# Jeremy-Cleland/hmer-img2latex

Measured on AMD Instinct MI355X. Metric: decoded LaTeX tokens/sec at batch 256, 320x64 imgs, seq 150, higher is better.
Workload: dtype f32

## Files before the change

hmer-img2latex_amd/csrc/conv_bf16x3.hip:

```cpp
#include <stdlib.h>

#include "common.h"

namespace {

#include "bf16_split.inc.h"

typedef float f32x16 __attribute__((ext_vector_type(16)));

constexpr int CH = 16;
constexpr int CO_BLK = 64;
constexpr int W_SLAB_U4 = 9 * 3 * 2 * CO_BLK;
constexpr int W_PHASE_U4 = W_SLAB_U4 / 3;

template <int WX> struct Tile3 {
    static constexpr int TR = (4 / WX) * 4, TC = WX * 16;
    static constexpr int IR = TR + 2, IC = TC + 2;
    static constexpr int ICP = WX == 2 ? 36 : (WX == 1 ? 20 : 68);
    static constexpr int ROW16 = 2 * ICP;
    static constexpr int IN_U4 = 3 * IR * ROW16;
};

constexpr unsigned FIX_HDR = 64;
constexpr unsigned FIX_CAP = 1u << 20;
constexpr float FIX_TOL = 0x1p-13f;

__device__ __forceinline__ void pool_window(float a0, float a1, float a2, float a3, float bv, float& outv, int& bi, bool& near) {
    float best = a0;
    bi = 0;
    if (a1 > best) { best = a1; bi = 1; }
    if (a2 > best) { best = a2; bi = 2; }
    if (a3 > best) { best = a3; bi = 3; }
    const float pre = best + bv;
    outv = fmaxf(pre, 0.f);
    const float scale = fmaxf(fmaxf(fabsf(best), fabsf(bv)), 1e-30f);
    const float thr = FIX_TOL * scale;
    const float d0 = best - a0, d1 = best - a1, d2 = best - a2, d3 = best - a3;
    const bool tie = (d0 > 0.f && d0 <= thr) || (d1 > 0.f && d1 <= thr) || (d2 > 0.f && d2 <= thr) || (d3 > 0.f && d3 <= thr);
    near = fabsf(pre) <= thr || (tie && pre > 0.f);
}
__device__ __forceinline__ void fix_append(unsigned* fix, size_t o) {
    const unsigned at = atomicAdd(fix, 1u);
    if (at < FIX_CAP) fix[FIX_HDR + at] = (unsigned)o;
}

__global__ void conv_pack3_kernel(const float* __restrict__ w, bf16_t* __restrict__ wp, int Cin, int Cout, int n_chunks,
                                  size_t total, int flip, unsigned* __restrict__ fix) {
    const size_t idx = (size_t)blockIdx.x * blockDim.x + threadIdx.x;
    if (idx == 0 && fix) fix[0] = 0;
    if (idx >= total) return;
    size_t r = idx;
    const int j = (int)(r % 8); r /= 8;
    const int co_l = (int)(r % CO_BLK); r /= CO_BLK;
    const int lh = (int)(r % 2); r /= 2;
    const int tap = (int)(r % 9); r /= 9;
    const int chunk = (int)(r % n_chunks);
    const int cb = (int)(r / n_chunks);
    const int co = cb * CO_BLK + co_l, ci = chunk * CH + 8 * lh + j;
    const float v = (co < Cout && ci < Cin) ? (flip ? w[((size_t)ci * Cout + co) * 9 + (8 - tap)] : w[((size_t)co * Cin + ci) * 9 + tap]) : 0.f;
    bf16_t s[3];
    split3(v, s[0], s[1], s[2]);
    const size_t slab = ((size_t)cb * n_chunks + chunk) * (size_t)W_SLAB_U4 * 8;
#pragma unroll
    for (int sp = 0; sp < 3; ++sp)
        wp[slab + ((((size_t)tap * 3 + sp) * 2 + lh) * CO_BLK + co_l) * 8 + j] = s[sp];
}

template <int WX, bool FULL = false, bool AM = false, int NT = 2>
__global__ __launch_bounds__(256, 2) void conv3x3_bf16x3_kernel(
    const float* __restrict__ x, const bf16_t* __restrict__ wpack, const float* __restrict__ bias,
    float* __restrict__ y, unsigned char* __restrict__ amax, int Cin, int H, int W, int Cout, int Hp, int Wp,
    int tiles_x, int n_chunks, int tiles_per_img, int n_items, int items_per_wg, unsigned* __restrict__ fix) {
    typedef Tile3<WX> TL;
    constexpr int PR = TL::TR / 2, PC = TL::TC / 2;
    constexpr bool LO = FULL && NT == 1;
    __shared__ __attribute__((aligned(16))) uint4 in_s[TL::IN_U4];
    __shared__ __attribute__((aligned(16))) uint4 w_s[W_PHASE_U4];
    __shared__ float out_s[CO_BLK * 65];
    __shared__ unsigned char am_s[AM ? CO_BLK * 68 : 4];

    const int tid = threadIdx.x, lane = tid & 63, wave = tid >> 6;
    const int wy = wave / WX, wx = wave % WX;
    constexpr int CO_W = 32 * NT;
    const int co_blocks_g = (Cout + CO_W - 1) / CO_W;
    const int lin = blockIdx.x, within = lin % (8 * co_blocks_g);
    const int cb = within >> 3;
    const int walk = (lin / (8 * co_blocks_g)) * 8 + (within & 7);
    const int i = lane & 31, h = lane >> 5;
    const int dx = i & 1, dy = (i >> 1) & 1, pp = i >> 2;
    const int a_base = ((wy * 4 + dy) * 2 + h) * TL::ICP + wx * 16 + 2 * pp + dx;
    const int b_base = h * CO_BLK + i + (NT == 1 ? (cb & 1) * 32 : 0);
    const uint4* wp_cb = reinterpret_cast<const uint4*>(wpack) + (size_t)(NT == 1 ? cb >> 1 : cb) * n_chunks * W_SLAB_U4;
    const int HW = H * W;

    constexpr int NP = TL::IR * 2 * TL::IC;
    constexpr int NE = (NP + 255) / 256;
    constexpr int NWV = (W_PHASE_U4 + 255) / 256;
    constexpr int SPLIT_U4 = TL::IR * TL::ROW16;
    int loff[NE], p_r[NE], p_col[NE], p_lh[NE];
#pragma unroll
    for (int e = 0; e < NE; ++e) {
        const int idx = tid + e * 256;
        p_col[e] = idx % TL::IC;
        p_lh[e] = (idx / TL::IC) & 1;
        p_r[e] = idx / (2 * TL::IC);
        loff[e] = idx < NP ? (p_r[e] * 2 + p_lh[e]) * TL::ICP + p_col[e] : -1;
    }
    const float* f_xb = x;
    int goff[NE];
    unsigned okmask = 0;
    auto setup_fetch = [&](int item) {
        const int fb = item / tiles_per_img, ft = item - fb * tiles_per_img;
        const int fty = ft / tiles_x, ftx = ft - fty * tiles_x;
        const int fy0 = fty * TL::TR, fx0 = ftx * TL::TC;
        f_xb = x + (size_t)fb * Cin * HW;
        okmask = 0;
#pragma unroll
        for (int e = 0; e < NE; ++e) {
            const int iy = fy0 - 1 + p_r[e], ix = fx0 - 1 + p_col[e];
            goff[e] = (8 * p_lh[e] * H + iy) * W + ix;
            if (loff[e] >= 0 && iy >= 0 && iy < H && ix >= 0 && ix < W) okmask |= 1u << e;
        }
    };
    float xin[NE][8];
    uint4 win[NWV];
    auto fetch_x = [&](int chunk) {
        const float* xc = f_xb + (size_t)chunk * CH * HW;
#pragma unroll
        for (int e = 0; e < NE; ++e) {
            const bool ok = (okmask >> e) & 1u;
#pragma unroll
            for (int j = 0; j < 8; ++j) xin[e][j] = ok ? xc[goff[e] + j * HW] : 0.f;
        }
    };
    auto fetch_w = [&](int phase) {
        const uint4* wsrc = wp_cb + (size_t)phase * W_PHASE_U4;
#pragma unroll
        for (int e = 0; e < NWV; ++e) {
            const int idx = tid + e * 256;
            win[e] = idx < W_PHASE_U4 ? wsrc[idx] : make_uint4(0, 0, 0, 0);
        }
    };
    auto commit_x = [&]() {
#pragma unroll
        for (int e = 0; e < NE; ++e) {
            if (loff[e] >= 0) {
                unsigned s[3][4];
#pragma unroll
                for (int j = 0; j < 4; ++j) split3_pair(xin[e][2 * j], xin[e][2 * j + 1], s[0][j], s[1][j], s[2][j]);
#pragma unroll
                for (int sp = 0; sp < 3; ++sp)
                    in_s[loff[e] + sp * SPLIT_U4] = make_uint4(s[sp][0], s[sp][1], s[sp][2], s[sp][3]);
            }
        }
    };
    auto commit_w = [&]() {
#pragma unroll
        for (int e = 0; e < NWV; ++e) {
            const int idx = tid + e * 256;
            if (idx < W_PHASE_U4) w_s[idx] = win[e];
        }
    };

    const int n_phases = 3 * n_chunks;
    const int it0 = walk * items_per_wg, it_end = min(it0 + items_per_wg, n_items);
    if (it0 >= n_items) return;
    setup_fetch(it0);
    fetch_x(0);
    fetch_w(0);
    for (int it = it0; it < it_end; ++it) {
        const int b = it / tiles_per_img, tl = it - b * tiles_per_img;
        const int ty = tl / tiles_x, tx = tl - ty * tiles_x;
        const int y0 = ty * TL::TR, x0 = tx * TL::TC;
        f32x16 acc[2][NT];
        f32x16 acc_lo[LO ? 2 : 1];
#pragma unroll
        for (int m = 0; m < 2; ++m)
#pragma unroll
            for (int n = 0; n < NT; ++n)
#pragma unroll
                for (int r = 0; r < 16; ++r) acc[m][n][r] = 0.f;
        if constexpr (LO) {
#pragma unroll
            for (int m = 0; m < 2; ++m)
#pragma unroll
                for (int r = 0; r < 16; ++r) acc_lo[m][r] = 0.f;
        }

        for (int chunk = 0; chunk < n_chunks; ++chunk) {
#pragma unroll
            for (int ky = 0; ky < 3; ++ky) {
                __syncthreads();
                if (ky == 0) commit_x();
                commit_w();
                __syncthreads();
                if (chunk * 3 + ky + 1 < n_phases) fetch_w(chunk * 3 + ky + 1);
                else if (it + 1 < it_end) fetch_w(0);
                if (ky == 0) {
                    if (chunk + 1 < n_chunks) fetch_x(chunk + 1);
                    else if (it + 1 < it_end) { setup_fetch(it + 1); fetch_x(0); }
                }
#pragma unroll
                for (int kx = 0; kx < 3; ++kx) {
                    i16x8_t a[2][3], bw[NT][3];
#pragma unroll
                    for (int m = 0; m < 2; ++m)
#pragma unroll
                        for (int sp = 0; sp < 3; ++sp) {
                            const uint4 t = in_s[a_base + (sp * TL::IR + m * 2 + ky) * TL::ROW16 + kx];
                            a[m][sp] = *reinterpret_cast<const i16x8_t*>(&t);
                        }
#pragma unroll
                    for (int n = 0; n < NT; ++n)
#pragma unroll
                        for (int sp = 0; sp < 3; ++sp) {
                            const uint4 t = w_s[b_base + ((kx * 3 + sp) * 2) * CO_BLK + n * 32];
                            bw[n][sp] = *reinterpret_cast<const i16x8_t*>(&t);
                        }
                    constexpr int TI[6] = {0, 1, 2, 0, 1, 0}, TJ[6] = {2, 1, 0, 1, 0, 0};
#pragma unroll
                    for (int t = 0; t < 6; ++t)
#pragma unroll
                        for (int m = 0; m < 2; ++m)
#pragma unroll
                            for (int n = 0; n < NT; ++n) {
                                if constexpr (LO) {
                                    f32x16& dst = t < 5 ? acc_lo[m] : acc[m][n];
                                    dst = __builtin_amdgcn_mfma_f32_32x32x16_bf16(a[m][TI[t]], bw[n][TJ[t]], dst, 0, 0, 0);
                                } else {
                                    acc[m][n] = __builtin_amdgcn_mfma_f32_32x32x16_bf16(a[m][TI[t]], bw[n][TJ[t]], acc[m][n], 0, 0, 0);
                                }
                            }
                }
            }
        }

        const int py0 = y0 >> 1, px0 = x0 >> 1;
        if constexpr (LO) {
#pragma unroll
            for (int m = 0; m < 2; ++m) acc[m][0] += acc_lo[m];
        }
        if constexpr (FULL) {
#pragma unroll
            for (int n = 0; n < NT; ++n) {
                const int co = cb * CO_W + n * 32 + i;
                if (co >= Cout) continue;
#pragma unroll
                for (int m = 0; m < 2; ++m) {
                    const int py = py0 + wy * 2 + m;
#pragma unroll
                    for (int q = 0; q < 4; ++q) {
                        const int px = px0 + wx * 8 + 2 * q + h;
#pragma unroll
                        for (int ry = 0; ry < 2; ++ry) {
                            const int Y = 2 * py + ry, X = 2 * px;
                            if (Y < H && X + 1 < W)
                                *reinterpret_cast<float2*>(y + (((size_t)b * Cout + co) * H + Y) * W + X) =
                                    make_float2(acc[m][n][4 * q + 2 * ry], acc[m][n][4 * q + 2 * ry + 1]);
                        }
                    }
                }
            }
            continue;
        }
        if ((Wp & 3) == 0 && py0 + PR <= Hp && px0 + PC <= Wp && (cb + 1) * CO_BLK <= Cout) {
#pragma unroll
            for (int n = 0; n < NT; ++n) {
                const float bv = bias[cb * CO_BLK + n * 32 + i];
#pragma unroll
                for (int m = 0; m < 2; ++m)
#pragma unroll
                    for (int q = 0; q < 4; ++q) {
                        const int pos = (wy * 2 + m) * PC + wx * 8 + 2 * q + h;
                        if constexpr (AM) {
                            float ov;
                            int bi;
                            bool near;
                            pool_window(acc[m][n][4 * q], acc[m][n][4 * q + 1], acc[m][n][4 * q + 2], acc[m][n][4 * q + 3], bv, ov, bi, near);
                            out_s[(n * 32 + i) * 65 + pos] = ov;
                            am_s[(n * 32 + i) * 68 + pos] = (unsigned char)bi;
                            if (near && fix)
                                fix_append(fix, (((size_t)b * Cout + cb * CO_BLK + n * 32 + i) * Hp + py0 + wy * 2 + m) * Wp + px0 + wx * 8 + 2 * q + h);
                        } else {
                            const float v = fmaxf(fmaxf(acc[m][n][4 * q], acc[m][n][4 * q + 1]),
                                                  fmaxf(acc[m][n][4 * q + 2], acc[m][n][4 * q + 3])) + bv;
                            out_s[(n * 32 + i) * 65 + pos] = fmaxf(v, 0.f);
                        }
                    }
            }
            __syncthreads();
            for (int idx = tid; idx < CO_BLK * 16; idx += 256) {
                constexpr int XG = PC / 4;
                const int x4 = idx % XG, py = (idx / XG) % PR, co_l = idx >> 4;
                const float* sp = &out_s[co_l * 65 + py * PC + 4 * x4];
                const size_t o = (((size_t)b * Cout + cb * CO_BLK + co_l) * Hp + py0 + py) * Wp + px0 + 4 * x4;
                *reinterpret_cast<float4*>(y + o) = make_float4(sp[0], sp[1], sp[2], sp[3]);
                if constexpr (AM) *reinterpret_cast<uchar4*>(amax + o) = *reinterpret_cast<const uchar4*>(&am_s[co_l * 68 + py * PC + 4 * x4]);
            }
            continue;
        }
#pragma unroll
        for (int n = 0; n < NT; ++n) {
            const int co = cb * CO_BLK + n * 32 + i;
            if (co >= Cout) continue;
            const float bv = bias[co];
#pragma unroll
            for (int m = 0; m < 2; ++m) {
                const int py = py0 + wy * 2 + m;
                if (py >= Hp) continue;
                const size_t rowoff = (((size_t)b * Cout + co) * Hp + py) * Wp;
#pragma unroll
                for (int q = 0; q < 4; ++q) {
                    const int px = px0 + wx * 8 + 2 * q + h;
                    float ov;
                    int bi;
                    bool near;
                    pool_window(acc[m][n][4 * q], acc[m][n][4 * q + 1], acc[m][n][4 * q + 2], acc[m][n][4 * q + 3], bv, ov, bi, near);
                    if (px < Wp) {
                        y[rowoff + px] = ov;
                        if (amax) amax[rowoff + px] = (unsigned char)bi;
                        if (AM && near && fix) fix_append(fix, rowoff + px);
                    }
                }
            }
        }
    }
}


template <int CIN, bool AM = false>
__global__ __launch_bounds__(256, 4) void conv3x3_smallk_bf16x3_kernel(
    const float* __restrict__ x, const float* __restrict__ w, const float* __restrict__ bias, float* __restrict__ y,
    unsigned char* __restrict__ amax, int H, int W, int Cout, int Hp, int Wp, int tiles_x, int tiles_per_part,
    unsigned* __restrict__ fix) {
    constexpr int RS = 48;
    constexpr int PLANE = 10 * RS;
    __shared__ __attribute__((aligned(16))) uint2 img[3 * PLANE];
    __shared__ float out_s[32 * 65];
    __shared__ unsigned char am_s[AM ? 32 * 68 : 4];

    const int tid = threadIdx.x, lane = tid & 63, wave = tid >> 6;
    const int wy = wave >> 1, wx = wave & 1;
    const int i = lane & 31, h = lane >> 5;
    const int cbs = (Cout + 31) / 32;
    const int cb = blockIdx.x % cbs, b = blockIdx.z;
    const int tx_begin = (blockIdx.x / cbs) * tiles_per_part, tx_end = min(tiles_x, tx_begin + tiles_per_part);
    const int y0 = blockIdx.y * 8;

    i16x8_t bw[3][3];
    {
        const int co = cb * 32 + i;
#pragma unroll
        for (int s = 0; s < 3; ++s) {
            unsigned pk[3][4];
#pragma unroll
            for (int j = 0; j < 4; ++j) {
                const int tap = 4 * s + 2 * h + (j >> 1), c0 = 2 * (j & 1);
                const bool okt = tap < 9 && co < Cout;
                const float v0 = (okt && c0 < CIN) ? w[((size_t)co * CIN + c0) * 9 + tap] : 0.f;
                const float v1 = (okt && c0 + 1 < CIN) ? w[((size_t)co * CIN + c0 + 1) * 9 + tap] : 0.f;
                split3_pair(v0, v1, pk[0][j], pk[1][j], pk[2][j]);
            }
#pragma unroll
            for (int sp = 0; sp < 3; ++sp) {
                const uint4 t = make_uint4(pk[sp][0], pk[sp][1], pk[sp][2], pk[sp][3]);
                bw[s][sp] = *reinterpret_cast<const i16x8_t*>(&t);
            }
        }
    }
    const float bv = (cb * 32 + i < Cout) ? bias[cb * 32 + i] : 0.f;

    const int pbase = (wy * 4 + ((i >> 1) & 1)) * RS + wx * 16 + 2 * (i >> 2) + (i & 1);
    int aoff[3][2];
#pragma unroll
    for (int s = 0; s < 3; ++s)
#pragma unroll
        for (int e = 0; e < 2; ++e) {
            const int tap = min(4 * s + 2 * h + e, 8);
            aoff[s][e] = pbase + (tap / 3) * RS + (tap % 3);
        }

    const float* xb = x + (size_t)b * CIN * H * W;
    const size_t HW = (size_t)H * W;
    int q_lds[2], q_col[2];
    long q_goff[2];
    bool q_rowok[2];
#pragma unroll
    for (int e = 0; e < 2; ++e) {
        const int q = tid + e * 256;
        const int r = q / 34, col = q - r * 34;
        const int iy = y0 - 1 + r;
        q_lds[e] = q < 340 ? r * RS + col : -1;
        q_col[e] = col - 1;
        q_rowok[e] = q < 340 && iy >= 0 && iy < H;
        q_goff[e] = (long)iy * W + col - 1;
    }
    float pin[2][CIN];
    auto fetch = [&](int tx) {
        const int x0 = tx * 32;
#pragma unroll
        for (int e = 0; e < 2; ++e) {
            const int ix = x0 + q_col[e];
            const bool ok = q_rowok[e] && ix >= 0 && ix < W;
#pragma unroll
            for (int c = 0; c < CIN; ++c) pin[e][c] = ok ? xb[c * HW + q_goff[e] + x0] : 0.f;
        }
    };
    fetch(tx_begin);
    for (int tx = tx_begin; tx < tx_end; ++tx) {
#pragma unroll
        for (int e = 0; e < 2; ++e) {
            if (q_lds[e] >= 0) {
                unsigned p0[3], p1[3];
                split3_pair(pin[e][0], CIN > 1 ? pin[e][CIN > 1 ? 1 : 0] : 0.f, p0[0], p0[1], p0[2]);
                split3_pair(CIN > 2 ? pin[e][CIN > 2 ? 2 : 0] : 0.f, 0.f, p1[0], p1[1], p1[2]);
#pragma unroll
                for (int sp = 0; sp < 3; ++sp) img[sp * PLANE + q_lds[e]] = make_uint2(p0[sp], p1[sp]);
            }
        }
        __syncthreads();
        if (tx + 1 < tx_end) fetch(tx + 1);
#pragma unroll 1
        for (int m = 0; m < 2; ++m) {
            f32x16 acc;
#pragma unroll
            for (int r = 0; r < 16; ++r) acc[r] = 0.f;
            constexpr int TI[5] = {0, 1, 2, 0, 1}, TJ[5] = {2, 1, 0, 1, 0};
            i16x8_t a0[3];
#pragma unroll
            for (int s = 0; s < 3; ++s) {
                i16x8_t a[3];
#pragma unroll
                for (int sp = 0; sp < 3; ++sp) {
                    const uint2 t0 = img[sp * PLANE + m * 2 * RS + aoff[s][0]];
                    const uint2 t1 = img[sp * PLANE + m * 2 * RS + aoff[s][1]];
                    const uint4 t = make_uint4(t0.x, t0.y, t1.x, t1.y);
                    a[sp] = *reinterpret_cast<const i16x8_t*>(&t);
                }
                a0[s] = a[0];
#pragma unroll
                for (int t = 0; t < 5; ++t)
                    acc = __builtin_amdgcn_mfma_f32_32x32x16_bf16(a[TI[t]], bw[s][TJ[t]], acc, 0, 0, 0);
            }
#pragma unroll
            for (int s = 0; s < 3; ++s) acc = __builtin_amdgcn_mfma_f32_32x32x16_bf16(a0[s], bw[s][0], acc, 0, 0, 0);
#pragma unroll
            for (int q = 0; q < 4; ++q) {
                const int pos = (wy * 2 + m) * 16 + wx * 8 + 2 * q + h;
                if constexpr (AM) {
                    float ov;
                    int bi;
                    bool near;
                    pool_window(acc[4 * q], acc[4 * q + 1], acc[4 * q + 2], acc[4 * q + 3], bv, ov, bi, near);
                    out_s[i * 65 + pos] = ov;
                    am_s[i * 68 + pos] = (unsigned char)bi;
                    const int fpy = (y0 >> 1) + wy * 2 + m, fpx = tx * 16 + wx * 8 + 2 * q + h;
                    if (near && fix && cb * 32 + i < Cout && fpy < Hp && fpx < Wp)
                        fix_append(fix, (((size_t)b * Cout + cb * 32 + i) * Hp + fpy) * Wp + fpx);
                } else {
                    const float v = fmaxf(fmaxf(acc[4 * q], acc[4 * q + 1]), fmaxf(acc[4 * q + 2], acc[4 * q + 3])) + bv;
                    out_s[i * 65 + pos] = fmaxf(v, 0.f);
                }
            }
        }
        __syncthreads();
        const int py0 = y0 >> 1, px0 = tx * 16;
        if ((Wp & 3) == 0 && py0 + 4 <= Hp && px0 + 16 <= Wp && (cb + 1) * 32 <= Cout) {
            for (int idx = tid; idx < 32 * 16; idx += 256) {
                const int x4 = idx & 3, py = (idx >> 2) & 3, c = idx >> 4;
                const float* sp = &out_s[c * 65 + py * 16 + 4 * x4];
                const size_t o = (((size_t)b * Cout + cb * 32 + c) * Hp + py0 + py) * Wp + px0 + 4 * x4;
                *reinterpret_cast<float4*>(y + o) = make_float4(sp[0], sp[1], sp[2], sp[3]);
                if constexpr (AM) *reinterpret_cast<uchar4*>(amax + o) = *reinterpret_cast<const uchar4*>(&am_s[c * 68 + py * 16 + 4 * x4]);
            }
        } else {
            for (int idx = tid; idx < 32 * 64; idx += 256) {
                const int px = idx & 15, py = (idx >> 4) & 3, c = idx >> 6;
                if (cb * 32 + c < Cout && py0 + py < Hp && px0 + px < Wp) {
                    const size_t o = (((size_t)b * Cout + cb * 32 + c) * Hp + py0 + py) * Wp + px0 + px;
                    y[o] = out_s[c * 65 + py * 16 + px];
                    if constexpr (AM) amax[o] = am_s[c * 68 + py * 16 + px];
                }
            }
        }
    }
}

__global__ __launch_bounds__(256) void conv_pool_fixup_kernel(const float* __restrict__ x, const float* __restrict__ w,
                                                              const float* __restrict__ bias, float* __restrict__ y,
                                                              unsigned char* __restrict__ amax, const unsigned* __restrict__ fix,
                                                              int Cin, int H, int W, int Cout, int Hp, int Wp) {
    const unsigned n = min(fix[0], FIX_CAP);
    const int lane = threadIdx.x & 63;
    for (unsigned e = blockIdx.x * 4 + (threadIdx.x >> 6); e < n; e += gridDim.x * 4) {
        const unsigned o = fix[FIX_HDR + e];
        const int px = (int)(o % Wp), py = (int)((o / Wp) % Hp);
        const int co = (int)((o / ((unsigned)Wp * Hp)) % Cout), b = (int)(o / ((unsigned)Wp * Hp * Cout));
        float s[4] = {0.f, 0.f, 0.f, 0.f};
        for (int ci = lane; ci < Cin; ci += 64) {
            const float* xp = x + ((size_t)b * Cin + ci) * H * W;
            const float* wp = w + ((size_t)co * Cin + ci) * 9;
            float win[4][4];
#pragma unroll
            for (int r = 0; r < 4; ++r)
#pragma unroll
                for (int c = 0; c < 4; ++c) {
                    const int iy = 2 * py - 1 + r, ix = 2 * px - 1 + c;
                    win[r][c] = (iy >= 0 && iy < H && ix >= 0 && ix < W) ? xp[(size_t)iy * W + ix] : 0.f;
                }
#pragma unroll
            for (int ky = 0; ky < 3; ++ky)
#pragma unroll
                for (int kx = 0; kx < 3; ++kx) {
                    const float wv = wp[ky * 3 + kx];
#pragma unroll
                    for (int q = 0; q < 4; ++q) s[q] = fmaf(win[(q >> 1) + ky][(q & 1) + kx], wv, s[q]);
                }
        }
#pragma unroll
        for (int q = 0; q < 4; ++q)
#pragma unroll
            for (int off = 32; off >= 1; off >>= 1) s[q] += __shfl_xor(s[q], off);
        if (lane == 0) {
            float best = s[0];
            int bi = 0;
#pragma unroll
            for (int q = 1; q < 4; ++q)
                if (s[q] > best) { best = s[q]; bi = q; }
            y[o] = fmaxf(best + bias[co], 0.f);
            amax[o] = (unsigned char)bi;
        }
    }
}

}

bool i2l_conv_bf16x3_applicable(int Cin, int Cout) {
    return Cin % CH == 0 && Cout % CO_BLK == 0;
}
bool i2l_conv_bf16x3_full_applicable(int Cin, int Cout) {
    return Cin % CH == 0 && (Cout % CO_BLK == 0 || Cout == 32);
}

size_t i2l_conv_bf16x3_workspace_bytes(int Cin, int Cout) {
    return i2l_align((size_t)((Cout + CO_BLK - 1) / CO_BLK) * (Cin / CH) * W_SLAB_U4 * 16);
}
size_t i2l_conv_fixlist_bytes(void) { return i2l_align((size_t)(FIX_HDR + FIX_CAP) * sizeof(unsigned)); }

namespace {
int launch_fixup(const float* x, const float* w, const float* bias, float* y, unsigned char* amax, const unsigned* fix,
                 int B, int Cin, int H, int W, int Cout, hipStream_t s) {
    if ((size_t)B * Cout * (H / 2) * (W / 2) > 0xffffffffull) return I2L_ERR_UNSUPPORTED;
    hipLaunchKernelGGL(conv_pool_fixup_kernel, dim3(512), dim3(256), 0, s, x, w, bias, y, amax, fix, Cin, H, W, Cout, H / 2, W / 2);
    I2L_CHECK_LAUNCH();
    return I2L_OK;
}
}

int i2l_conv_bf16x3_run(const float* x, const float* w, const float* bias, float* y, unsigned char* amax, int B, int Cin,
                        int H, int W, int Cout, void* workspace, size_t workspace_bytes, hipStream_t s, int full,
                        int weights_packed) {
    if (full && ((H | W) & 1)) return I2L_ERR_UNSUPPORTED;
    const size_t pack_bytes = i2l_conv_bf16x3_workspace_bytes(Cin, Cout);
    if (workspace_bytes < pack_bytes + (amax ? i2l_conv_fixlist_bytes() : 0) || !workspace) return I2L_ERR_WORKSPACE;
    unsigned* fix = amax ? reinterpret_cast<unsigned*>(static_cast<char*>(workspace) + pack_bytes) : nullptr;
    if (amax && (size_t)B * Cout * (H / 2) * (W / 2) > 0xffffffffull) return I2L_ERR_UNSUPPORTED;
    const int Hp = H / 2, Wp = W / 2;
    const int n_chunks = Cin / CH, co_blocks = (Cout + CO_BLK - 1) / CO_BLK;
    if (Cout % CO_BLK != 0 && !(full && Cout == 32)) return I2L_ERR_UNSUPPORTED;
    bf16_t* wp = static_cast<bf16_t*>(workspace);
    const size_t total = (size_t)co_blocks * n_chunks * 9 * 2 * CO_BLK * 8;
    if (!(weights_packed && !amax && !full))
    hipLaunchKernelGGL(conv_pack3_kernel, dim3((unsigned)((total + 255) / 256)), dim3(256), 0, s, w, wp, Cin, Cout,
                       n_chunks, total, full ? 1 : 0, fix);
    I2L_CHECK_LAUNCH();
    const int rows = 2 * Hp, cols = 2 * Wp;
    int wx = 2;
    long bestw = -1;
    const int cand[3] = {2, 1, 4};
    for (int c = 0; c < 3; ++c) {
        const int tr = (4 / cand[c]) * 4, tc = cand[c] * 16;
        const long cover = (long)i2l_cdiv(rows, tr) * tr * i2l_cdiv(cols, tc) * tc;
        if (bestw < 0 || cover < bestw) { bestw = cover; wx = cand[c]; }
    }
    const int tr = (4 / wx) * 4, tc = wx * 16;
    const int tiles_x = i2l_cdiv(cols, tc), tiles_y = i2l_cdiv(rows, tr);
    const int tiles_per_img = tiles_x * tiles_y;
    const long long n_items_ll = (long long)tiles_per_img * B;
    if (n_items_ll > 0x7fffffffll) return I2L_ERR_UNSUPPORTED;
    const int n_items = (int)n_items_ll;
    const int wg_blocks = full ? (Cout + 31) / 32 : co_blocks;
    int items_per_wg = (int)((n_items_ll * wg_blocks + 511) / 512);
    if (n_items_ll * wg_blocks <= 768) items_per_wg = 1;
    if (items_per_wg < 1) items_per_wg = 1;
    const int walks = i2l_cdiv(n_items, items_per_wg);
    dim3 grid((unsigned)(i2l_cdiv(walks, 8) * 8 * wg_blocks));
#define I2L_LAUNCH3(WXV)                                                                                              \
    do {                                                                                                              \
        if (full)                                                                                                     \
            hipLaunchKernelGGL((conv3x3_bf16x3_kernel<WXV, true, false, 1>), grid, dim3(256), 0, s, x, (const bf16_t*)wp, bias, y, \
                               amax, Cin, H, W, Cout, Hp, Wp, tiles_x, n_chunks, tiles_per_img, n_items, items_per_wg, fix); \
        else if (amax)                                                                                                \
            hipLaunchKernelGGL((conv3x3_bf16x3_kernel<WXV, false, true>), grid, dim3(256), 0, s, x, (const bf16_t*)wp, bias, y, \
                               amax, Cin, H, W, Cout, Hp, Wp, tiles_x, n_chunks, tiles_per_img, n_items, items_per_wg, fix); \
        else                                                                                                          \
            hipLaunchKernelGGL((conv3x3_bf16x3_kernel<WXV, false>), grid, dim3(256), 0, s, x, (const bf16_t*)wp, bias, y, \
                               amax, Cin, H, W, Cout, Hp, Wp, tiles_x, n_chunks, tiles_per_img, n_items, items_per_wg, fix); \
    } while (0)
    if (wx == 2) I2L_LAUNCH3(2);
    else if (wx == 1) I2L_LAUNCH3(1);
    else I2L_LAUNCH3(4);
#undef I2L_LAUNCH3
    I2L_CHECK_LAUNCH();
    if (amax) return launch_fixup(x, w, bias, y, amax, fix, B, Cin, H, W, Cout, s);
    return I2L_OK;
}

bool i2l_conv_smallk_applicable(int Cin, int Cout) {
    return Cin >= 1 && Cin <= 3 && Cout % 32 == 0;
}

int i2l_conv_smallk_run(const float* x, const float* w, const float* bias, float* y, unsigned char* amax, int B, int Cin,
                        int H, int W, int Cout, void* workspace, size_t workspace_bytes, hipStream_t s) {
    const int Hp = H / 2, Wp = W / 2;
    unsigned* fix = nullptr;
    if (amax) {
        if (!workspace || workspace_bytes < i2l_conv_fixlist_bytes()) return I2L_ERR_WORKSPACE;
        if ((size_t)B * Cout * Hp * Wp > 0xffffffffull) return I2L_ERR_UNSUPPORTED;
        fix = static_cast<unsigned*>(workspace);
        if (hipMemsetAsync(fix, 0, sizeof(unsigned), s) != hipSuccess) return I2L_ERR_LAUNCH;
    }
    const int tiles_x = i2l_cdiv(2 * Wp, 32), bands = i2l_cdiv(2 * Hp, 8);
    if (bands > 65535 || B > 65535) return I2L_ERR_UNSUPPORTED;
    int parts = 1;
    while (parts < tiles_x && (long)(Cout / 32) * bands * B * parts < 1536) ++parts;
    const int tiles_per_part = i2l_cdiv(tiles_x, parts);
    parts = i2l_cdiv(tiles_x, tiles_per_part);
    dim3 grid((Cout / 32) * parts, bands, B);
#define I2L_LAUNCH_SK(C, A) hipLaunchKernelGGL((conv3x3_smallk_bf16x3_kernel<C, A>), grid, dim3(256), 0, s, x, w, bias, y, amax, H, W, Cout, Hp, Wp, tiles_x, tiles_per_part, fix)
    if (amax) {
        if (Cin == 1) I2L_LAUNCH_SK(1, true);
        else if (Cin == 2) I2L_LAUNCH_SK(2, true);
        else I2L_LAUNCH_SK(3, true);
    } else {
        if (Cin == 1) I2L_LAUNCH_SK(1, false);
        else if (Cin == 2) I2L_LAUNCH_SK(2, false);
        else I2L_LAUNCH_SK(3, false);
    }
#undef I2L_LAUNCH_SK
    I2L_CHECK_LAUNCH();
    if (amax) return launch_fixup(x, w, bias, y, amax, fix, B, Cin, H, W, Cout, s);
    return I2L_OK;
}
```

Baseline: 41.22 million.

## Double-buffer first-layer small-K conv tiles and overlap staging with MFMA compute

Splits the small-K bf16x3 conv into separate argmax and plain kernels. The plain kernel double-buffers the LDS input image and the output staging tile. It commits the next tile and stores the previous tile's pooled outputs between the two MFMA m-tiles, with sched barriers, so it needs one __syncthreads per tile instead of two. Input addressing switches to 32-bit byte offsets to cut address math, and a guard is added for tensors that would overflow it. The cost is roughly double the LDS per block, which may lower occupancy below the launch-bounds target of 4 blocks.

```diff
diff --git a/hmer-img2latex_amd/csrc/conv_bf16x3.hip b/hmer-img2latex_amd/csrc/conv_bf16x3.hip
--- a/hmer-img2latex_amd/csrc/conv_bf16x3.hip
+++ b/hmer-img2latex_amd/csrc/conv_bf16x3.hip
@@ -328,16 +328,125 @@
 }
 
 
-template <int CIN, bool AM = false>
-__global__ __launch_bounds__(256, 4) void conv3x3_smallk_bf16x3_kernel(
+constexpr int SK_RS = 48;
+constexpr int SK_PLANE = 10 * SK_RS;
+constexpr int SK_IMG = 3 * SK_PLANE;
+constexpr int SK_OUT = 32 * 65;
+
+template <int CIN>
+__device__ __forceinline__ void smallk_filter_bank(const float* __restrict__ w, int co, int Cout, int h, i16x8_t (&bw)[3][3]) {
+#pragma unroll
+    for (int s = 0; s < 3; ++s) {
+        unsigned pk[3][4];
+#pragma unroll
+        for (int j = 0; j < 4; ++j) {
+            const int tap = 4 * s + 2 * h + (j >> 1), c0 = 2 * (j & 1);
+            const bool okt = tap < 9 && co < Cout;
+            const float v0 = (okt && c0 < CIN) ? w[((size_t)co * CIN + c0) * 9 + tap] : 0.f;
+            const float v1 = (okt && c0 + 1 < CIN) ? w[((size_t)co * CIN + c0 + 1) * 9 + tap] : 0.f;
+            split3_pair(v0, v1, pk[0][j], pk[1][j], pk[2][j]);
+        }
+#pragma unroll
+        for (int sp = 0; sp < 3; ++sp) {
+            const uint4 t = make_uint4(pk[sp][0], pk[sp][1], pk[sp][2], pk[sp][3]);
+            bw[s][sp] = *reinterpret_cast<const i16x8_t*>(&t);
+        }
+    }
+}
+
+__device__ __forceinline__ void smallk_a_offsets(int wy, int wx, int i, int h, int (&aoff)[3][2]) {
+    const int pbase = (wy * 4 + ((i >> 1) & 1)) * SK_RS + wx * 16 + 2 * (i >> 2) + (i & 1);
+#pragma unroll
+    for (int s = 0; s < 3; ++s)
+#pragma unroll
+        for (int e = 0; e < 2; ++e) {
+            const int tap = min(4 * s + 2 * h + e, 8);
+            aoff[s][e] = pbase + (tap / 3) * SK_RS + (tap % 3);
+        }
+}
+
+template <int CIN> struct SmallKStage {
+    const char* xb;
+    unsigned plane_bytes;
+    int W;
+    int q_lds[2], q_col[2];
+    unsigned q_boff[2];
+    bool q_rowok[2];
+    float pin[2][CIN];
+    __device__ __forceinline__ void init(const float* x_img, int H, int W_, int y0, int tid) {
+        xb = reinterpret_cast<const char*>(x_img);
+        plane_bytes = (unsigned)H * (unsigned)W_ * 4u;
+        W = W_;
+#pragma unroll
+        for (int e = 0; e < 2; ++e) {
+            const int q = tid + e * 256;
+            const int r = q / 34, col = q - r * 34;
+            const int iy = y0 - 1 + r;
+            q_lds[e] = q < 340 ? r * SK_RS + col : -1;
+            q_col[e] = col - 1;
+            q_rowok[e] = q < 340 && iy >= 0 && iy < H;
+            q_boff[e] = ((unsigned)iy * (unsigned)W_ + (unsigned)(col - 1)) * 4u;
+        }
+    }
+    __device__ __forceinline__ void fetch(int tx) {
+        const int x0 = tx * 32;
+#pragma unroll
+        for (int e = 0; e < 2; ++e) {
+            const int ix = x0 + q_col[e];
+            const bool ok = q_rowok[e] && ix >= 0 && ix < W;
+#pragma unroll
+            for (int c = 0; c < CIN; ++c)
+                pin[e][c] = ok ? *reinterpret_cast<const float*>(xb + (q_boff[e] + 4u * (unsigned)x0 + (unsigned)c * plane_bytes)) : 0.f;
+        }
+    }
+    __device__ __forceinline__ void commit(uint2* im) const {
+#pragma unroll
+        for (int e = 0; e < 2; ++e) {
+            if (q_lds[e] >= 0) {
+                unsigned p0[3], p1[3];
+                split3_pair(pin[e][0], CIN > 1 ? pin[e][CIN > 1 ? 1 : 0] : 0.f, p0[0], p0[1], p0[2]);
+                split3_pair(CIN > 2 ? pin[e][CIN > 2 ? 2 : 0] : 0.f, 0.f, p1[0], p1[1], p1[2]);
+#pragma unroll
+                for (int sp = 0; sp < 3; ++sp) im[sp * SK_PLANE + q_lds[e]] = make_uint2(p0[sp], p1[sp]);
+            }
+        }
+    }
+};
+
+__device__ __forceinline__ f32x16 smallk_mtile(const uint2* im, int moff, const int (&aoff)[3][2], const i16x8_t (&bw)[3][3]) {
+    f32x16 acc;
+#pragma unroll
+    for (int r = 0; r < 16; ++r) acc[r] = 0.f;
+    constexpr int TI[5] = {0, 1, 2, 0, 1}, TJ[5] = {2, 1, 0, 1, 0};
+    i16x8_t a0[3];
+#pragma unroll
+    for (int s = 0; s < 3; ++s) {
+        i16x8_t a[3];
+#pragma unroll
+        for (int sp = 0; sp < 3; ++sp) {
+            const uint2 t0 = im[sp * SK_PLANE + moff + aoff[s][0]];
+            const uint2 t1 = im[sp * SK_PLANE + moff + aoff[s][1]];
+            const uint4 t = make_uint4(t0.x, t0.y, t1.x, t1.y);
+            a[sp] = *reinterpret_cast<const i16x8_t*>(&t);
+        }
+        a0[s] = a[0];
+#pragma unroll
+        for (int t = 0; t < 5; ++t)
+            acc = __builtin_amdgcn_mfma_f32_32x32x16_bf16(a[TI[t]], bw[s][TJ[t]], acc, 0, 0, 0);
+    }
+#pragma unroll
+    for (int s = 0; s < 3; ++s) acc = __builtin_amdgcn_mfma_f32_32x32x16_bf16(a0[s], bw[s][0], acc, 0, 0, 0);
+    return acc;
+}
+
+template <int CIN>
+__global__ __launch_bounds__(256, 4) void conv3x3_smallk_bf16x3_kernel_am(
     const float* __restrict__ x, const float* __restrict__ w, const float* __restrict__ bias, float* __restrict__ y,
     unsigned char* __restrict__ amax, int H, int W, int Cout, int Hp, int Wp, int tiles_x, int tiles_per_part,
     unsigned* __restrict__ fix) {
-    constexpr int RS = 48;
-    constexpr int PLANE = 10 * RS;
-    __shared__ __attribute__((aligned(16))) uint2 img[3 * PLANE];
-    __shared__ float out_s[32 * 65];
-    __shared__ unsigned char am_s[AM ? 32 * 68 : 4];
+    __shared__ __attribute__((aligned(16))) uint2 img[SK_IMG];
+    __shared__ float out_s[SK_OUT];
+    __shared__ unsigned char am_s[32 * 68];
 
     const int tid = threadIdx.x, lane = tid & 63, wave = tid >> 6;
     const int wy = wave >> 1, wx = wave & 1;
@@ -348,119 +457,33 @@
     const int y0 = blockIdx.y * 8;
 
     i16x8_t bw[3][3];
-    {
-        const int co = cb * 32 + i;
-#pragma unroll
-        for (int s = 0; s < 3; ++s) {
-            unsigned pk[3][4];
-#pragma unroll
-            for (int j = 0; j < 4; ++j) {
-                const int tap = 4 * s + 2 * h + (j >> 1), c0 = 2 * (j & 1);
-                const bool okt = tap < 9 && co < Cout;
-                const float v0 = (okt && c0 < CIN) ? w[((size_t)co * CIN + c0) * 9 + tap] : 0.f;
-                const float v1 = (okt && c0 + 1 < CIN) ? w[((size_t)co * CIN + c0 + 1) * 9 + tap] : 0.f;
-                split3_pair(v0, v1, pk[0][j], pk[1][j], pk[2][j]);
-            }
-#pragma unroll
-            for (int sp = 0; sp < 3; ++sp) {
-                const uint4 t = make_uint4(pk[sp][0], pk[sp][1], pk[sp][2], pk[sp][3]);
-                bw[s][sp] = *reinterpret_cast<const i16x8_t*>(&t);
-            }
-        }
-    }
+    smallk_filter_bank<CIN>(w, cb * 32 + i, Cout, h, bw);
     const float bv = (cb * 32 + i < Cout) ? bias[cb * 32 + i] : 0.f;
-
-    const int pbase = (wy * 4 + ((i >> 1) & 1)) * RS + wx * 16 + 2 * (i >> 2) + (i & 1);
     int aoff[3][2];
-#pragma unroll
-    for (int s = 0; s < 3; ++s)
-#pragma unroll
-        for (int e = 0; e < 2; ++e) {
-            const int tap = min(4 * s + 2 * h + e, 8);
-            aoff[s][e] = pbase + (tap / 3) * RS + (tap % 3);
-        }
-
-    const float* xb = x + (size_t)b * CIN * H * W;
-    const size_t HW = (size_t)H * W;
-    int q_lds[2], q_col[2];
-    long q_goff[2];
-    bool q_rowok[2];
-#pragma unroll
-    for (int e = 0; e < 2; ++e) {
-        const int q = tid + e * 256;
-        const int r = q / 34, col = q - r * 34;
-        const int iy = y0 - 1 + r;
-        q_lds[e] = q < 340 ? r * RS + col : -1;
-        q_col[e] = col - 1;
-        q_rowok[e] = q < 340 && iy >= 0 && iy < H;
-        q_goff[e] = (long)iy * W + col - 1;
-    }
-    float pin[2][CIN];
-    auto fetch = [&](int tx) {
-        const int x0 = tx * 32;
-#pragma unroll
-        for (int e = 0; e < 2; ++e) {
-            const int ix = x0 + q_col[e];
-            const bool ok = q_rowok[e] && ix >= 0 && ix < W;
-#pragma unroll
-            for (int c = 0; c < CIN; ++c) pin[e][c] = ok ? xb[c * HW + q_goff[e] + x0] : 0.f;
-        }
-    };
-    fetch(tx_begin);
+    smallk_a_offsets(wy, wx, i, h, aoff);
+    SmallKStage<CIN> st;
+    st.init(x + (size_t)b * CIN * H * W, H, W, y0, tid);
+
+    st.fetch(tx_begin);
     for (int tx = tx_begin; tx < tx_end; ++tx) {
-#pragma unroll
-        for (int e = 0; e < 2; ++e) {
-            if (q_lds[e] >= 0) {
-                unsigned p0[3], p1[3];
-                split3_pair(pin[e][0], CIN > 1 ? pin[e][CIN > 1 ? 1 : 0] : 0.f, p0[0], p0[1], p0[2]);
-                split3_pair(CIN > 2 ? pin[e][CIN > 2 ? 2 : 0] : 0.f, 0.f, p1[0], p1[1], p1[2]);
-#pragma unroll
-                for (int sp = 0; sp < 3; ++sp) img[sp * PLANE + q_lds[e]] = make_uint2(p0[sp], p1[sp]);
-            }
-        }
+        st.commit(img);
         __syncthreads();
-        if (tx + 1 < tx_end) fetch(tx + 1);
+        if (tx + 1 < tx_end) st.fetch(tx + 1);
 #pragma unroll 1
         for (int m = 0; m < 2; ++m) {
-            f32x16 acc;
-#pragma unroll
-            for (int r = 0; r < 16; ++r) acc[r] = 0.f;
-            constexpr int TI[5] = {0, 1, 2, 0, 1}, TJ[5] = {2, 1, 0, 1, 0};
-            i16x8_t a0[3];
-#pragma unroll
-            for (int s = 0; s < 3; ++s) {
-                i16x8_t a[3];
-#pragma unroll
-                for (int sp = 0; sp < 3; ++sp) {
-                    const uint2 t0 = img[sp * PLANE + m * 2 * RS + aoff[s][0]];
-                    const uint2 t1 = img[sp * PLANE + m * 2 * RS + aoff[s][1]];
-                    const uint4 t = make_uint4(t0.x, t0.y, t1.x, t1.y);
-                    a[sp] = *reinterpret_cast<const i16x8_t*>(&t);
-                }
-                a0[s] = a[0];
-#pragma unroll
-                for (int t = 0; t < 5; ++t)
-                    acc = __builtin_amdgcn_mfma_f32_32x32x16_bf16(a[TI[t]], bw[s][TJ[t]], acc, 0, 0, 0);
-            }
-#pragma unroll
-            for (int s = 0; s < 3; ++s) acc = __builtin_amdgcn_mfma_f32_32x32x16_bf16(a0[s], bw[s][0], acc, 0, 0, 0);
+            const f32x16 acc = smallk_mtile(img, m * 2 * SK_RS, aoff, bw);
 #pragma unroll
             for (int q = 0; q < 4; ++q) {
                 const int pos = (wy * 2 + m) * 16 + wx * 8 + 2 * q + h;
-                if constexpr (AM) {
-                    float ov;
-                    int bi;
-                    bool near;
-                    pool_window(acc[4 * q], acc[4 * q + 1], acc[4 * q + 2], acc[4 * q + 3], bv, ov, bi, near);
-                    out_s[i * 65 + pos] = ov;
-                    am_s[i * 68 + pos] = (unsigned char)bi;
-                    const int fpy = (y0 >> 1) + wy * 2 + m, fpx = tx * 16 + wx * 8 + 2 * q + h;
-                    if (near && fix && cb * 32 + i < Cout && fpy < Hp && fpx < Wp)
-                        fix_append(fix, (((size_t)b * Cout + cb * 32 + i) * Hp + fpy) * Wp + fpx);
-                } else {
-                    const float v = fmaxf(fmaxf(acc[4 * q], acc[4 * q + 1]), fmaxf(acc[4 * q + 2], acc[4 * q + 3])) + bv;
-                    out_s[i * 65 + pos] = fmaxf(v, 0.f);
-                }
+                float ov;
+                int bi;
+                bool near;
+                pool_window(acc[4 * q], acc[4 * q + 1], acc[4 * q + 2], acc[4 * q + 3], bv, ov, bi, near);
+                out_s[i * 65 + pos] = ov;
+                am_s[i * 68 + pos] = (unsigned char)bi;
+                const int fpy = (y0 >> 1) + wy * 2 + m, fpx = tx * 16 + wx * 8 + 2 * q + h;
+                if (near && fix && cb * 32 + i < Cout && fpy < Hp && fpx < Wp)
+                    fix_append(fix, (((size_t)b * Cout + cb * 32 + i) * Hp + fpy) * Wp + fpx);
             }
         }
         __syncthreads();
@@ -471,7 +494,7 @@
                 const float* sp = &out_s[c * 65 + py * 16 + 4 * x4];
                 const size_t o = (((size_t)b * Cout + cb * 32 + c) * Hp + py0 + py) * Wp + px0 + 4 * x4;
                 *reinterpret_cast<float4*>(y + o) = make_float4(sp[0], sp[1], sp[2], sp[3]);
-                if constexpr (AM) *reinterpret_cast<uchar4*>(amax + o) = *reinterpret_cast<const uchar4*>(&am_s[c * 68 + py * 16 + 4 * x4]);
+                *reinterpret_cast<uchar4*>(amax + o) = *reinterpret_cast<const uchar4*>(&am_s[c * 68 + py * 16 + 4 * x4]);
             }
         } else {
             for (int idx = tid; idx < 32 * 64; idx += 256) {
@@ -479,11 +502,86 @@
                 if (cb * 32 + c < Cout && py0 + py < Hp && px0 + px < Wp) {
                     const size_t o = (((size_t)b * Cout + cb * 32 + c) * Hp + py0 + py) * Wp + px0 + px;
                     y[o] = out_s[c * 65 + py * 16 + px];
-                    if constexpr (AM) amax[o] = am_s[c * 68 + py * 16 + px];
+                    amax[o] = am_s[c * 68 + py * 16 + px];
                 }
             }
         }
     }
+}
+
+template <int CIN>
+__global__ __launch_bounds__(256, 4) void conv3x3_smallk_bf16x3_kernel(
+    const float* __restrict__ x, const float* __restrict__ w, const float* __restrict__ bias, float* __restrict__ y,
+    int H, int W, int Cout, int Hp, int Wp, int tiles_x, int tiles_per_part) {
+    __shared__ __attribute__((aligned(16))) uint2 img[2 * SK_IMG];
+    __shared__ float out_s[2 * SK_OUT];
+
+    const int tid = threadIdx.x, lane = tid & 63, wave = tid >> 6;
+    const int wy = wave >> 1, wx = wave & 1;
+    const int i = lane & 31, h = lane >> 5;
+    const int cbs = (Cout + 31) / 32;
+    const int cb = blockIdx.x % cbs, b = blockIdx.z;
+    const int tx_begin = (blockIdx.x / cbs) * tiles_per_part, tx_end = min(tiles_x, tx_begin + tiles_per_part);
+    const int y0 = blockIdx.y * 8;
+
+    i16x8_t bw[3][3];
+    smallk_filter_bank<CIN>(w, cb * 32 + i, Cout, h, bw);
+    const float bv = (cb * 32 + i < Cout) ? bias[cb * 32 + i] : 0.f;
+    int aoff[3][2];
+    smallk_a_offsets(wy, wx, i, h, aoff);
+    SmallKStage<CIN> st;
+    st.init(x + (size_t)b * CIN * H * W, H, W, y0, tid);
+
+    const int py0 = y0 >> 1;
+    const bool whole_rows = (Wp & 3) == 0 && py0 + 4 <= Hp && (cb + 1) * 32 <= Cout;
+    auto pool = [&](const f32x16& acc, float* os, int m) {
+#pragma unroll
+        for (int q = 0; q < 4; ++q) {
+            const int pos = (wy * 2 + m) * 16 + wx * 8 + 2 * q + h;
+            const float v = fmaxf(fmaxf(acc[4 * q], acc[4 * q + 1]), fmaxf(acc[4 * q + 2], acc[4 * q + 3])) + bv;
+            os[i * 65 + pos] = fmaxf(v, 0.f);
+        }
+    };
+    auto store = [&](const float* os, int tx) {
+        const int px0 = tx * 16;
+        if (whole_rows && px0 + 16 <= Wp) {
+#pragma unroll
+            for (int idx = tid; idx < 32 * 16; idx += 256) {
+                const int x4 = idx & 3, py = (idx >> 2) & 3, c = idx >> 4;
+                const float* sp = &os[c * 65 + py * 16 + 4 * x4];
+                const size_t o = (((size_t)b * Cout + cb * 32 + c) * Hp + py0 + py) * Wp + px0 + 4 * x4;
+                *reinterpret_cast<float4*>(y + o) = make_float4(sp[0], sp[1], sp[2], sp[3]);
+            }
+        } else {
+            for (int idx = tid; idx < 32 * 64; idx += 256) {
+                const int px = idx & 15, py = (idx >> 4) & 3, c = idx >> 6;
+                if (cb * 32 + c < Cout && py0 + py < Hp && px0 + px < Wp)
+                    y[(((size_t)b * Cout + cb * 32 + c) * Hp + py0 + py) * Wp + px0 + px] = os[c * 65 + py * 16 + px];
+            }
+        }
+    };
+
+    if (tx_begin >= tx_end) return;
+    st.fetch(tx_begin);
+    st.commit(img);
+    if (tx_begin + 1 < tx_end) st.fetch(tx_begin + 1);
+    __syncthreads();
+    for (int tx = tx_begin; tx < tx_end; ++tx) {
+        const int p = (tx - tx_begin) & 1;
+        const uint2* im = img + p * SK_IMG;
+        float* os = out_s + p * SK_OUT;
+        pool(smallk_mtile(im, 0, aoff, bw), os, 0);
+        __builtin_amdgcn_sched_barrier(0);
+        if (tx + 1 < tx_end) {
+            st.commit(img + (p ^ 1) * SK_IMG);
+            if (tx + 2 < tx_end) st.fetch(tx + 2);
+        }
+        if (tx > tx_begin) store(out_s + (p ^ 1) * SK_OUT, tx - 1);
+        __builtin_amdgcn_sched_barrier(0);
+        pool(smallk_mtile(im + 2 * SK_RS, 0, aoff, bw), os, 1);
+        __syncthreads();
+    }
+    store(out_s + ((tx_end - 1 - tx_begin) & 1) * SK_OUT, tx_end - 1);
 }
 
 __global__ __launch_bounds__(256) void conv_pool_fixup_kernel(const float* __restrict__ x, const float* __restrict__ w,
@@ -632,22 +730,25 @@
     }
     const int tiles_x = i2l_cdiv(2 * Wp, 32), bands = i2l_cdiv(2 * Hp, 8);
     if (bands > 65535 || B > 65535) return I2L_ERR_UNSUPPORTED;
+    if ((size_t)Cin * H * W * sizeof(float) > 0xffffffffull) return I2L_ERR_UNSUPPORTED;
     int parts = 1;
     while (parts < tiles_x && (long)(Cout / 32) * bands * B * parts < 1536) ++parts;
     const int tiles_per_part = i2l_cdiv(tiles_x, parts);
     parts = i2l_cdiv(tiles_x, tiles_per_part);
     dim3 grid((Cout / 32) * parts, bands, B);
-#define I2L_LAUNCH_SK(C, A) hipLaunchKernelGGL((conv3x3_smallk_bf16x3_kernel<C, A>), grid, dim3(256), 0, s, x, w, bias, y, amax, H, W, Cout, Hp, Wp, tiles_x, tiles_per_part, fix)
+#define I2L_LAUNCH_SK_AM(C) hipLaunchKernelGGL((conv3x3_smallk_bf16x3_kernel_am<C>), grid, dim3(256), 0, s, x, w, bias, y, amax, H, W, Cout, Hp, Wp, tiles_x, tiles_per_part, fix)
+#define I2L_LAUNCH_SK(C) hipLaunchKernelGGL((conv3x3_smallk_bf16x3_kernel<C>), grid, dim3(256), 0, s, x, w, bias, y, H, W, Cout, Hp, Wp, tiles_x, tiles_per_part)
     if (amax) {
-        if (Cin == 1) I2L_LAUNCH_SK(1, true);
-        else if (Cin == 2) I2L_LAUNCH_SK(2, true);
-        else I2L_LAUNCH_SK(3, true);
+        if (Cin == 1) I2L_LAUNCH_SK_AM(1);
+        else if (Cin == 2) I2L_LAUNCH_SK_AM(2);
+        else I2L_LAUNCH_SK_AM(3);
     } else {
-        if (Cin == 1) I2L_LAUNCH_SK(1, false);
-        else if (Cin == 2) I2L_LAUNCH_SK(2, false);
-        else I2L_LAUNCH_SK(3, false);
+        if (Cin == 1) I2L_LAUNCH_SK(1);
+        else if (Cin == 2) I2L_LAUNCH_SK(2);
+        else I2L_LAUNCH_SK(3);
     }
 #undef I2L_LAUNCH_SK
+#undef I2L_LAUNCH_SK_AM
     I2L_CHECK_LAUNCH();
     if (amax) return launch_fixup(x, w, bias, y, amax, fix, B, Cin, H, W, Cout, s);
     return I2L_OK;
diff --git a/profiles/conv_first_cost.py b/profiles/conv_first_cost.py
--- /dev/null
+++ b/profiles/conv_first_cost.py
@@ -0,0 +1,148 @@
+import collections
+import csv
+import ctypes
+import os
+import statistics
+import sys
+
+KERNEL = "conv3x3_smallk_bf16x3_kernel<3"
+DECODE = "decode_group16_kernel"
+FLAGSHIP = (256, 3, 64, 320, 32)
+TEST_SHAPES = [(B, cin, H, W, Cout) for (B, H, W, Cout) in
+               ((48, 64, 96, 128), (2, 10, 70, 32), (2, 7, 9, 32), (2, 16, 34, 32), (2, 16, 64, 32), (2, 16, 64, 64))
+               for cin in (1, 2, 3)]
+
+
+def _load(path):
+    L = ctypes.CDLL(os.path.abspath(path))
+    L.i2l_conv_workspace_bytes.restype = ctypes.c_size_t
+    L.i2l_conv_workspace_bytes.argtypes = [ctypes.c_int, ctypes.c_int]
+    L.i2l_conv3x3_relu_pool2_fwd.restype = ctypes.c_int
+    L.i2l_conv3x3_relu_pool2_fwd.argtypes = [ctypes.c_void_p] * 5 + [ctypes.c_int] * 5 + [ctypes.c_void_p, ctypes.c_size_t,
+                                                                                      ctypes.c_int, ctypes.c_void_p]
+    return L
+
+
+def micro(other):
+    import torch
+    here = os.path.join(os.path.dirname(os.path.abspath(__file__)), "..", "hmer-img2latex_amd", "img2latex_amd",
+                        "libimg2latex_hip.so")
+    libs = {"parent": _load(other), "this": _load(here)}
+    stream = torch.cuda.current_stream().cuda_stream
+
+    def run(L, ops, case, y):
+        B, Cin, H, W, Cout = case
+        nb = L.i2l_conv_workspace_bytes(Cin, Cout)
+        ws = torch.empty(max(nb, 16), dtype=torch.uint8, device="cuda")
+        rc = L.i2l_conv3x3_relu_pool2_fwd(ops[0].data_ptr(), ops[1].data_ptr(), ops[2].data_ptr(), y.data_ptr(), None,
+                                          B, Cin, H, W, Cout, ws.data_ptr(), nb, 0, stream)
+        assert rc == 0, (case, rc)
+
+    def operands(case, seed):
+        B, Cin, H, W, Cout = case
+        g = torch.Generator().manual_seed(seed)
+        return (torch.randn(B, Cin, H, W, generator=g).cuda(),
+                (torch.randn(Cout, Cin, 3, 3, generator=g) / (3 * Cin ** 0.5)).cuda(), torch.randn(Cout, generator=g).cuda())
+
+    print("1. bit identity of i2l_conv3x3_relu_pool2_fwd (flags 0, no arg max), parent build against this build")
+    all_equal = True
+    for n, case in enumerate([FLAGSHIP] + TEST_SHAPES):
+        B, Cin, H, W, Cout = case
+        ops = operands(case, 900 + n)
+        ys = {}
+        for name, L in libs.items():
+            y = torch.full((B, Cout, H // 2, W // 2), float("nan"), device="cuda")
+            run(L, ops, case, y)
+            torch.cuda.synchronize()
+            ys[name] = y
+        eq = torch.equal(ys["parent"], ys["this"]) and bool(torch.isfinite(ys["this"]).all())
+        all_equal &= eq
+        print(f"   {case}: {'torch.equal' if eq else 'DIFFERENT'}")
+    print(f"   all equal: {all_equal}")
+
+    print("2. the flagship launch alone on the chip, us (median / min / max of 30 launches per round, 3 alternating rounds)")
+    _time(libs, run, operands)
+    return 0 if all_equal else 1
+
+
+def _time(libs, run, operands):
+    import torch
+    ops = operands(FLAGSHIP, 900)
+    B, Cin, H, W, Cout = FLAGSHIP
+    y = torch.empty((B, Cout, H // 2, W // 2), device="cuda")
+    for rnd in range(3):
+        for name, L in libs.items():
+            for _ in range(5):
+                run(L, ops, FLAGSHIP, y)
+            ts = []
+            for _ in range(30):
+                e0, e1 = torch.cuda.Event(enable_timing=True), torch.cuda.Event(enable_timing=True)
+                e0.record()
+                run(L, ops, FLAGSHIP, y)
+                e1.record()
+                e1.synchronize()
+                ts.append(e0.elapsed_time(e1) * 1e3)
+            print(f"   round {rnd + 1} {name:6s}  {statistics.median(ts):7.1f} / {min(ts):7.1f} / {max(ts):7.1f}")
+
+
+def trace(paths):
+    for path in paths:
+        conv, dec = [], []
+        for r in csv.DictReader(open(path)):
+            name = r["Kernel_Name"]
+            if KERNEL in name:
+                conv.append((int(r["Start_Timestamp"]), int(r["End_Timestamp"])))
+            elif DECODE in name:
+                dec.append((int(r["Start_Timestamp"]), int(r["End_Timestamp"])))
+        dec.sort()
+        groups = collections.defaultdict(list)
+        for s, e in conv:
+            inside = any(ds <= s and e <= de for ds, de in dec)
+            touch = any(ds < e and s < de for ds, de in dec)
+            groups["beside the decode (wholly inside a decode launch)" if inside else
+                   "partly beside" if touch else "alone"].append((e - s) / 1e3)
+        print(f"{path}: {len(conv)} launches of {KERNEL}..>")
+        for k, v in sorted(groups.items()):
+            v.sort()
+            print(f"   {k:52s} n = {len(v):4d}  mean {statistics.mean(v):6.1f}  median {statistics.median(v):6.1f}  "
+                  f"p10 {v[len(v) // 10]:6.1f}  p90 {v[(9 * len(v)) // 10]:6.1f}  min {v[0]:6.1f}  max {v[-1]:6.1f} us")
+    return 0
+
+
+def pmc(path):
+    sums, counts = collections.defaultdict(float), collections.Counter()
+    for r in csv.DictReader(open(path)):
+        if KERNEL in r["Kernel_Name"]:
+            sums[r["Counter_Name"]] += float(r["Counter_Value"])
+            counts[r["Counter_Name"]] += 1
+    for k in sorted(sums):
+        print(f"   {k:28s} {sums[k] / counts[k]:16.0f} per launch ({counts[k]} launches)")
+    if "SQ_WAVE_CYCLES" in sums:
+        wc = sums["SQ_WAVE_CYCLES"]
+        for k in ("SQ_WAIT_ANY", "SQ_WAIT_INST_ANY", "SQ_ACTIVE_INST_ANY", "SQ_WAIT_INST_LDS"):
+            if k in sums:
+                print(f"   {k} / SQ_WAVE_CYCLES = {sums[k] / wc:.3f}")
+    return 0
+
+
+def ids(a, b):
+    import numpy as np
+    ok = True
+    for f in ("ids.npy", "ids_serial.npy"):
+        same = np.array_equal(np.load(os.path.join(a, f)), np.load(os.path.join(b, f)))
+        ok &= same
+        print(f"   {f}: {'identical' if same else 'DIFFERENT'}")
+    return 0 if ok else 1
+
+
+if __name__ == "__main__":
+    cmd = sys.argv[1] if len(sys.argv) > 1 else ""
+    if cmd == "micro":
+        sys.exit(micro(sys.argv[2]))
+    if cmd == "trace":
+        sys.exit(trace(sys.argv[2:]))
+    if cmd == "pmc":
+        sys.exit(pmc(sys.argv[2]))
+    if cmd == "ids":
+        sys.exit(ids(sys.argv[2], sys.argv[3]))
+    sys.exit(__doc__)
```

Result: no change. 41.35 million (median of 6 runs) (+0.3%).
